# wendongbi/Bridged-GNN

Measured on AMD Instinct MI355X. Metric: aggregated_edges_per_sec_ktgnn_fwd, higher is better.
Workload: dtype f32; 1 GPU; C4 synthetic bridged graph (local) N=1000000 E'=20991058, 2-layer KT-GNN eval fwd F=128 hidden=128 C=2; parallelism=single, execution=eager launches

## Files before the change

bridged_gnn_amd/csrc/bgnn_transform_cls.hip:

```cpp
#include <cstdio>
#include <cstdlib>
#include "bgnn_common.h"
#include "bgnn_transform_params.h"

using bgnn_tf::GemmParams;
using bgnn_tf::MAXH;
using bgnn_tf::f32x16;
using bgnn_tf::tanh_fast;

namespace {

typedef _Float16 h8 __attribute__((ext_vector_type(8)));
typedef _Float16 h4 __attribute__((ext_vector_type(4)));

constexpr int CLS_TARGET_EXP = 10;
constexpr int DK = 128, KB16 = DK / 16, NCT = 4;
constexpr int PIECE = 32 * DK * 2;
constexpr int SLOT = 32 * 36 * 4 + 2 * 32 * 4;
constexpr int T_LD = 36;

__device__ __forceinline__ int chunk_off(int r, int c) { return r * 256 + ((c ^ (r & 15)) << 4); }
__device__ __forceinline__ void pow2_scales(float mx, float& sc, float& inv) {
  int E = (__builtin_bit_cast(int, mx) >> 23) & 0xff;
  E = E < 40 ? 40 : E;
  sc = __builtin_bit_cast(float, (127 + CLS_TARGET_EXP + 127 - E) << 23);
  inv = __builtin_bit_cast(float, (E - CLS_TARGET_EXP) << 23);
}

constexpr int CLS_NW = 4;

__global__ __launch_bounds__(64 * CLS_NW) void cls_stage_kernel(GemmParams p) {
  __shared__ __attribute__((aligned(16))) unsigned char wl[(NCT + 1) * 2 * PIECE];
  __shared__ __attribute__((aligned(16))) unsigned char slots[CLS_NW * SLOT];
  __shared__ __attribute__((aligned(16))) h8 w2lds[NCT][2][2][64];
  __shared__ __attribute__((aligned(16))) float skc[2][32];
  __shared__ __attribute__((aligned(16))) float bias1[DK];
  __shared__ uint32_t wmax[3];
  __shared__ float red[2][DK + 1];
  const int tid = threadIdx.x, lane = tid & 63;
  const int wave = __builtin_amdgcn_readfirstlane(tid >> 6);
  const int fr = lane & 31, fh = lane >> 5;
  const int NC = p.NC;
  const bool din_full = p.Din == DK;
#ifdef CLS_STAMP
  uint32_t st_acc[8] = {0, 0, 0, 0, 0, 0, 0, 0};
  uint32_t st_last = 0;
#define CLS_MARK(k) do { const uint32_t t__ = (uint32_t)__builtin_amdgcn_s_memtime(); st_acc[k] += t__ - st_last; st_last = t__; } while (0)
#else
#define CLS_MARK(k) do { } while (0)
#endif

  if (tid < 3) wmax[tid] = 0u;
  for (int t = tid; t < 2 * (DK + 1); t += 64 * CLS_NW) (&red[0][0])[t] = 0.f;
  if (tid < 32) { skc[0][tid] = tid < p.sk_NC ? p.sk_bias[tid] : 0.f; skc[1][tid] = tid < p.sk_NC ? p.sk_wd[tid] : 0.f; }
  if (tid < DK) bias1[tid] = tid < NC ? p.bias[tid] : 0.f;
  __syncthreads();
  auto src_row = [&](int ct, int r) -> const float* {
    if (ct < NCT) return (32 * ct + r) < NC ? p.Wp + (int64_t)(32 * ct + r) * p.Din : nullptr;
    if (r < p.sk_NC) return p.sk_Wp + (int64_t)r * p.Din;
    if (r >= 24 && ((r - 24) & 3) < 2 * p.sk_heads) return p.sk_g + (int64_t)((r - 24) & 3) * 2 * p.Din;
    return nullptr;
  };
  float mx1 = 0.f, mxs = 0.f;
  for (int it = tid; it < (NCT + 1) * 32 * 16; it += 64 * CLS_NW) {
    const int ct = it / 512, r = (it >> 4) & 31, c = it & 15;
    const float* s = src_row(ct, r);
    float m = 0.f;
    if (s != nullptr) {
#pragma unroll
      for (int e = 0; e < 8; ++e) { const int k = 8 * c + e; m = fmaxf(m, k < p.Din ? fabsf(s[k]) : 0.f); }
    }
    if (ct < NCT) mx1 = fmaxf(mx1, m); else mxs = fmaxf(mxs, m);
  }
  float w2v[NCT][16];
  float mx2 = 0.f;
#pragma unroll
  for (int ct = 0; ct < NCT; ++ct)
#pragma unroll
    for (int r = 0; r < 16; ++r) {
      const int c = 32 * ct + 8 * (r >> 2) + 4 * fh + (r & 3);
      float v = 0.f;
      if (c < NC) {
        if (fr < 8) v = p.w2[(int64_t)fr * NC + c];
        else if (fr < 10) v = p.g2[(int64_t)(fr - 8) * 2 * NC + c];
      }
      w2v[ct][r] = v;
      mx2 = fmaxf(mx2, fabsf(v));
    }
  mx1 = bgnn::group_max<64>(mx1); mxs = bgnn::group_max<64>(mxs); mx2 = bgnn::group_max<64>(mx2);
  if (lane == 0) {
    atomicMax(&wmax[0], __builtin_bit_cast(unsigned, mx1));
    atomicMax(&wmax[1], __builtin_bit_cast(unsigned, mxs));
    atomicMax(&wmax[2], __builtin_bit_cast(unsigned, mx2));
  }
  __syncthreads();
  float scW, cinvW, scS, cinvS, sc2w, cinv2;
  pow2_scales(__builtin_bit_cast(float, wmax[0]), scW, cinvW);
  pow2_scales(__builtin_bit_cast(float, wmax[1]), scS, cinvS);
  pow2_scales(__builtin_bit_cast(float, wmax[2]), sc2w, cinv2);
  for (int it = tid; it < (NCT + 1) * 32 * 16; it += 64 * CLS_NW) {
    const int ct = it / 512, r = (it >> 4) & 31, c = it & 15;
    const float* s = src_row(ct, r);
    const float sc = ct < NCT ? scW : scS;
    h8 hi, lo;
#pragma unroll
    for (int e = 0; e < 8; ++e) {
      const int k = 8 * c + e;
      const float v = (s != nullptr && k < p.Din) ? s[k] : 0.f;
      const _Float16 h = (_Float16)(v * sc);
      hi[e] = h;
      lo[e] = (_Float16)fmaf(v, sc, -(float)h);
    }
    unsigned char* base = wl + (ct * 2) * PIECE + chunk_off(r, c);
    *reinterpret_cast<h8*>(base) = hi;
    *reinterpret_cast<h8*>(base + PIECE) = lo;
  }
  if (wave == 0) {
#pragma unroll
    for (int ct = 0; ct < NCT; ++ct) {
      h8 hh[2], ll[2];
#pragma unroll
      for (int r = 0; r < 16; ++r) {
        const _Float16 h = (_Float16)(w2v[ct][r] * sc2w);
        hh[r >> 3][r & 7] = h;
        ll[r >> 3][r & 7] = (_Float16)fmaf(w2v[ct][r], sc2w, -(float)h);
      }
#pragma unroll
      for (int kb = 0; kb < 2; ++kb) { w2lds[ct][kb][0][lane] = hh[kb]; w2lds[ct][kb][1][lane] = ll[kb]; }
    }
  }
  __syncthreads();

  float* optr[3];
  int hsel[3];
#pragma unroll
  for (int q = 0; q < 3; ++q) {
    const int c = 8 * q + 4 * fh;
    optr[q] = nullptr; hsel[q] = 0;
    if (c < p.sk_NC) {
      const int ld2 = 2 * (int)p.sk_ldh;
      const int h = c / ld2, rem = c % ld2, t = rem >= p.sk_ldh ? 1 : 0;
      float* base = h == 0 ? (t == 0 ? p.sk_out[0][0] : p.sk_out[0][1]) : (t == 0 ? p.sk_out[1][0] : p.sk_out[1][1]);
      optr[q] = base + (rem - t * (int)p.sk_ldh);
      hsel[q] = h * 2 + t;
    }
  }
  float gcs[4];
#pragma unroll
  for (int h = 0; h < 4; ++h) gcs[h] = h < 2 * p.sk_heads ? p.sk_gc[h] : 0.f;

  unsigned char* const sb = slots + wave * SLOT;
  float* const tsc = reinterpret_cast<float*>(sb);
  float* const cfs = reinterpret_cast<float*>(sb + 32 * T_LD * 4);
  const int roff0 = chunk_off(fr, fh);
  auto roff = [&](int kb) { return roff0 ^ (kb << 5); };
  const int64_t ntiles = (p.N + 31) / 32;
  const int64_t stride = (int64_t)gridDim.x * CLS_NW;
  int64_t tile = (int64_t)blockIdx.x * CLS_NW + wave;
  float4 ra[KB16][2];
  uint8_t rmk = 0;
  auto gload = [&](int64_t tl) {
    int64_t r = tl * 32 + fr;
    r = r < p.N ? r : p.N - 1;
    const float* src = p.x + r * p.ldx;
#pragma unroll
    for (int kb = 0; kb < KB16; ++kb)
#pragma unroll
      for (int c = 0; c < 2; ++c) {
        const int k = 16 * kb + 8 * fh + 4 * c;
        ra[kb][c] = *reinterpret_cast<const float4*>(src + (din_full || k < p.Din ? k : 0));
      }
    rmk = p.mask[r];
  };
  float cs_s[NCT], cs_t[NCT], cnt_s = 0.f, cnt_t = 0.f;
#pragma unroll
  for (int ct = 0; ct < NCT; ++ct) cs_s[ct] = cs_t[ct] = 0.f;

  if (tile < ntiles) gload(tile);
  for (; tile < ntiles; tile += stride) {
    CLS_MARK(0);
    const bool sdom = rmk != 0;
    const int64_t row = tile * 32 + fr;
    const bool valid = row < p.N;
    float mx = 0.f;
#pragma unroll
    for (int kb = 0; kb < KB16; ++kb)
#pragma unroll
      for (int c = 0; c < 2; ++c) {
        if (!din_full && 16 * kb + 8 * fh + 4 * c >= p.Din) ra[kb][c] = make_float4(0.f, 0.f, 0.f, 0.f);
        mx = fmaxf(fmaxf(fabsf(ra[kb][c].x), fabsf(ra[kb][c].y)), mx);
        mx = fmaxf(fmaxf(fabsf(ra[kb][c].z), fabsf(ra[kb][c].w)), mx);
      }
    mx = fmaxf(mx, __shfl_xor(mx, 32));
    float scx, s_row;
    pow2_scales(mx, scx, s_row);
    h8 xh[KB16], xl[KB16];
#pragma unroll
    for (int kb = 0; kb < KB16; ++kb)
#pragma unroll
      for (int c = 0; c < 2; ++c) {
        const float f[4] = {ra[kb][c].x, ra[kb][c].y, ra[kb][c].z, ra[kb][c].w};
#pragma unroll
        for (int e = 0; e < 4; ++e) {
          const _Float16 h = (_Float16)(f[e] * scx);
          xh[kb][4 * c + e] = h;
          xl[kb][4 * c + e] = (_Float16)fmaf(f[e], scx, -(float)h);
        }
      }
    const float dom = sdom ? 1.f : 0.f;
    if (fh == 0) {
      cfs[fr] = (valid && sdom) ? 1.f : 0.f;
      cfs[32 + fr] = (valid && !sdom) ? 1.f : 0.f;
      cnt_s += (valid && sdom) ? 1.f : 0.f;
      cnt_t += (valid && !sdom) ? 1.f : 0.f;
    }
    const int64_t tnext = tile + stride < ntiles ? tile + stride : tile;
    gload(tnext);
    __builtin_amdgcn_fence(__ATOMIC_RELEASE, "workgroup", "local");
    constexpr int HK = KB16 / 2;
    h8 wf[2][HK][2];
    auto fetch_w = [&](int hc, int buf) {
      const int op = hc >> 1, half = hc & 1;
      const unsigned char* wb = wl + ((op == 0 ? NCT : op - 1) * 2) * PIECE;
#pragma unroll
      for (int j = 0; j < HK; ++j) {
        wf[buf][j][0] = *reinterpret_cast<const h8*>(wb + roff(HK * half + j));
        wf[buf][j][1] = *reinterpret_cast<const h8*>(wb + PIECE + roff(HK * half + j));
      }
    };
    auto half_chain = [&](int hc, f32x16& acc, auto&& between) {
      if (hc + 1 < 2 * (NCT + 1)) fetch_w(hc + 1, (hc + 1) & 1);
      __builtin_amdgcn_sched_barrier(0);
      const int half = hc & 1, buf = hc & 1;
#pragma unroll
      for (int j = 0; j < HK; ++j) {
        const int kb = HK * half + j;
        acc = __builtin_amdgcn_mfma_f32_32x32x16_f16(wf[buf][j][0], xl[kb], acc, 0, 0, 0);
        acc = __builtin_amdgcn_mfma_f32_32x32x16_f16(wf[buf][j][1], xh[kb], acc, 0, 0, 0);
        acc = __builtin_amdgcn_mfma_f32_32x32x16_f16(wf[buf][j][0], xh[kb], acc, 0, 0, 0);
        between(kb);
      }
    };
    auto nothing = [](int) {};
    CLS_MARK(1);
    fetch_w(0, 0);
    {
      f32x16 acc;
#pragma unroll
      for (int r = 0; r < 16; ++r) acc[r] = 0.f;
      half_chain(0, acc, nothing);
      half_chain(1, acc, nothing);
      CLS_MARK(2);
      const float ss = s_row * cinvS;
      if (valid) {
        float cf = 0.f;
#pragma unroll
        for (int q = 0; q < 3; ++q) {
          if (optr[q] != nullptr) {
            if (q == 0 || hsel[q] != hsel[q - 1]) {
              const bool t1 = hsel[q] & 1;
              const float pre = hsel[q] == 0 ? acc[12] : hsel[q] == 1 ? acc[13] : hsel[q] == 2 ? acc[14] : acc[15];
              const float gcv = hsel[q] == 0 ? gcs[0] : hsel[q] == 1 ? gcs[1] : hsel[q] == 2 ? gcs[2] : gcs[3];
              cf = ((dom != 0.f) != t1) ? tanh_fast(fmaf(pre, ss, gcv)) : 0.f;
              cf = t1 ? cf : -cf;
            }
            const float4 bq = *reinterpret_cast<const float4*>(&skc[0][8 * q + 4 * fh]), wq = *reinterpret_cast<const float4*>(&skc[1][8 * q + 4 * fh]);
            float4 o;
            o.x = fmaf(cf, wq.x, fmaf(acc[4 * q], ss, bq.x));     o.y = fmaf(cf, wq.y, fmaf(acc[4 * q + 1], ss, bq.y));
            o.z = fmaf(cf, wq.z, fmaf(acc[4 * q + 2], ss, bq.z)); o.w = fmaf(cf, wq.w, fmaf(acc[4 * q + 3], ss, bq.w));
            *reinterpret_cast<float4*>(optr[q] + row * p.sk_row_stride) = o;
          }
        }
      }
    }
    float o2[8];
#pragma unroll
    for (int i = 0; i < 8; ++i) o2[i] = 0.f;
    const float sc1 = s_row * cinvW;
    struct Stage2 { float a1[16]; float mx, sc2, inv2; h8 ah[2], al[2]; f32x16 acc2; h8 w2h[2], w2l[2]; };
    auto stage2_step = [&](Stage2& q, int ct, int j) {
      if (j == 0) {
        q.mx = fmaxf(q.mx, __shfl_xor(q.mx, 32));
#pragma unroll
        for (int kb = 0; kb < 2; ++kb) { q.w2h[kb] = w2lds[ct][kb][0][lane]; q.w2l[kb] = w2lds[ct][kb][1][lane]; }
      } else if (j == 1) {
        pow2_scales(q.mx, q.sc2, q.inv2);
#pragma unroll
        for (int r = 0; r < 16; ++r) q.acc2[r] = 0.f;
      } else if (j == 2 || j == 3) {
        const int kb = j - 2;
#pragma unroll
        for (int e = 0; e < 8; ++e) {
          const _Float16 h = (_Float16)(q.a1[8 * kb + e] * q.sc2);
          q.ah[kb][e] = h;
          q.al[kb][e] = (_Float16)fmaf(q.a1[8 * kb + e], q.sc2, -(float)h);
        }
      } else if (j == 4 || j == 5) {
        const int kb = j - 4;
        q.acc2 = __builtin_amdgcn_mfma_f32_32x32x16_f16(q.w2h[kb], q.al[kb], q.acc2, 0, 0, 0);
        q.acc2 = __builtin_amdgcn_mfma_f32_32x32x16_f16(q.w2l[kb], q.ah[kb], q.acc2, 0, 0, 0);
        q.acc2 = __builtin_amdgcn_mfma_f32_32x32x16_f16(q.w2h[kb], q.ah[kb], q.acc2, 0, 0, 0);
      } else if (j == 6) {
#pragma unroll
        for (int r = 0; r < 16; ++r) {
          const float v = tsc[(16 * fh + r) * T_LD + fr];
          cs_s[ct] = fmaf(cfs[16 * fh + r], v, cs_s[ct]);
          cs_t[ct] = fmaf(cfs[32 + 16 * fh + r], v, cs_t[ct]);
        }
      } else {
        const float s2 = q.inv2 * cinv2;
#pragma unroll
        for (int i = 0; i < 8; ++i) o2[i] = fmaf(q.acc2[i], s2, o2[i]);
      }
    };
    Stage2 q2;
    f32x16 acc;
#pragma unroll
    for (int r = 0; r < 16; ++r) acc[r] = 0.f;
    CLS_MARK(3);
    half_chain(2, acc, nothing);
    half_chain(3, acc, nothing);
    CLS_MARK(4);
#pragma unroll
    for (int ct = 0; ct < NCT; ++ct) {
      __builtin_amdgcn_fence(__ATOMIC_RELEASE, "workgroup", "local");
      q2.mx = 0.f;
#pragma unroll
      for (int qq = 0; qq < 4; ++qq) {
        const float4 b4 = *reinterpret_cast<const float4*>(&bias1[32 * ct + 8 * qq + 4 * fh]);
        const float bb[4] = {b4.x, b4.y, b4.z, b4.w};
#pragma unroll
        for (int e = 0; e < 4; ++e) {
          float v = fmaf(acc[4 * qq + e], sc1, bb[e]);
          if (p.relu) v = fmaxf(v, 0.f);
          q2.a1[4 * qq + e] = v;
          q2.mx = fmaxf(q2.mx, fabsf(v));
        }
        *reinterpret_cast<float4*>(&tsc[fr * T_LD + 8 * qq + 4 * fh]) =
            make_float4(q2.a1[4 * qq], q2.a1[4 * qq + 1], q2.a1[4 * qq + 2], q2.a1[4 * qq + 3]);
      }
      CLS_MARK(5);
      if (ct + 1 < NCT) {
#pragma unroll
        for (int r = 0; r < 16; ++r) acc[r] = 0.f;
        half_chain(2 * (ct + 2), acc, [&](int kb) { stage2_step(q2, ct, kb); });
        half_chain(2 * (ct + 2) + 1, acc, [&](int kb) { stage2_step(q2, ct, kb); });
        CLS_MARK(6);
      } else {
#pragma unroll
        for (int j = 0; j < 8; ++j) stage2_step(q2, ct, j);
        CLS_MARK(7);
      }
    }
    if (valid) {
      float* rr = p.raw + row * 12;
      if (fh == 0) {
        *reinterpret_cast<float4*>(rr) = make_float4(o2[0], o2[1], o2[2], o2[3]);
        *reinterpret_cast<float4*>(rr + 8) = make_float4(o2[4], o2[5], 0.f, 0.f);
      } else {
        *reinterpret_cast<float4*>(rr + 4) = make_float4(o2[0], o2[1], o2[2], o2[3]);
      }
    }
  }
#ifdef CLS_STAMP
  if (lane == 0 && p.wd != nullptr) {
    float* o = const_cast<float*>(p.wd) + ((int64_t)blockIdx.x * CLS_NW + wave) * 8;
    for (int k = 0; k < 8; ++k) o[k] = (float)st_acc[k];
  }
  return;
#endif
  if (p.colsum != nullptr) {
#pragma unroll
    for (int ct = 0; ct < NCT; ++ct) {
      const float a = cs_s[ct] + __shfl_xor(cs_s[ct], 32), b = cs_t[ct] + __shfl_xor(cs_t[ct], 32);
      if (fh == 0) {
        unsafeAtomicAdd(&red[0][32 * ct + fr], a);
        unsafeAtomicAdd(&red[1][32 * ct + fr], b);
      }
    }
    {
      float a = cnt_s, b = cnt_t;
#pragma unroll
      for (int m = 32; m >= 1; m >>= 1) { a += __shfl_xor(a, m); b += __shfl_xor(b, m); }
      if (lane == 0) { unsafeAtomicAdd(&red[0][DK], a); unsafeAtomicAdd(&red[1][DK], b); }
    }
    __syncthreads();
    for (int t = tid; t < 2 * (DK + 1); t += 64 * CLS_NW) {
      const int d = t / (DK + 1), c = t % (DK + 1);
      const double v = (double)red[d][c];
      if (c == DK) unsafeAtomicAdd(&p.colsum[2 * NC + d], v);
      else if (c < NC) unsafeAtomicAdd(&p.colsum[d * NC + c], v);
    }
  }
}

}

bool bgnn_tf_cls_supported(const GemmParams& p) {
  if (p.NC != 128 || p.Din > 128 || p.Din <= 64 || (p.Din & 3) || !p.mask || !p.w2 || !p.g2 || !p.raw) return false;
  if (p.sk_NC < 0 || p.sk_NC > 24 || (p.sk_NC & 3) || p.sk_heads < 0 || p.sk_heads > 2) return false;
  if (p.sk_NC > 0 && (!p.sk_Wp || !p.sk_bias || !p.sk_wd || !p.sk_g || !p.sk_gc || (p.sk_ldh & 3) || p.sk_NC != p.sk_heads * 2 * p.sk_ldh)) return false;
  return true;
}

int bgnn_tf_cls_launch(const GemmParams& p, hipStream_t st, int n_cu) {
  if (!bgnn_tf_cls_supported(p)) return BGNN_E_SHAPE;
  const int64_t nt = (p.N + 31) / 32, nb = (nt + CLS_NW - 1) / CLS_NW;
#ifdef CLS_STAMP
  {
    GemmParams q = p;
    static float* dbuf = nullptr;
    if (!dbuf) (void)hipMalloc((void**)&dbuf, sizeof(float) * 256 * 8 * 8);
    q.wd = dbuf;
    const unsigned g = (unsigned)(nb < n_cu ? nb : n_cu);
    hipLaunchKernelGGL(cls_stage_kernel, dim3(g), dim3(64 * CLS_NW), 0, st, q);
    (void)hipDeviceSynchronize();
    static float host[256 * 8 * 8];
    (void)hipMemcpy(host, dbuf, sizeof(float) * g * CLS_NW * 8, hipMemcpyDeviceToHost);
    double acc[8] = {0};
    for (unsigned w = 0; w < g * CLS_NW; ++w) for (int k = 0; k < 8; ++k) acc[k] += host[w * 8 + k];
    const double d = (double)nt;
    fprintf(stderr, "[cls stamp] cycles per tile: loop %.0f convert %.0f skinny-chain %.0f skinny-epilogue %.0f first-chain %.0f activation(x4) %.0f chain+stage2(x3) %.0f last-stage2 %.0f\n",
            acc[0] / d, acc[1] / d, acc[2] / d, acc[3] / d, acc[4] / d, acc[5] / d, acc[6] / d, acc[7] / d);
    return 0;
  }
#endif
  hipLaunchKernelGGL(cls_stage_kernel, dim3((unsigned)(nb < n_cu ? nb : n_cu)), dim3(64 * CLS_NW), 0, st, p);
  BGNN_LAUNCH_CHECK();
  return 0;
}
```

Measured before the change: 49.68 billion edges/s.

## Double waves per block and simplify cls pipeline to cut register pressure

Result: no change. 50.08 billion edges/s (median of 6 runs) (+0.8%).

```diff
diff --git a/bridged_gnn_amd/csrc/bgnn_transform_cls.hip b/bridged_gnn_amd/csrc/bgnn_transform_cls.hip
--- a/bridged_gnn_amd/csrc/bgnn_transform_cls.hip
+++ b/bridged_gnn_amd/csrc/bgnn_transform_cls.hip
@@ -27,7 +27,7 @@
   inv = __builtin_bit_cast(float, (E - CLS_TARGET_EXP) << 23);
 }
 
-constexpr int CLS_NW = 4;
+constexpr int CLS_NW = 8;
 
 __global__ __launch_bounds__(64 * CLS_NW) void cls_stage_kernel(GemmParams p) {
   __shared__ __attribute__((aligned(16))) unsigned char wl[(NCT + 1) * 2 * PIECE];
@@ -156,32 +156,28 @@
   auto roff = [&](int kb) { return roff0 ^ (kb << 5); };
   const int64_t ntiles = (p.N + 31) / 32;
   const int64_t stride = (int64_t)gridDim.x * CLS_NW;
-  int64_t tile = (int64_t)blockIdx.x * CLS_NW + wave;
-  float4 ra[KB16][2];
-  uint8_t rmk = 0;
-  auto gload = [&](int64_t tl) {
-    int64_t r = tl * 32 + fr;
-    r = r < p.N ? r : p.N - 1;
-    const float* src = p.x + r * p.ldx;
-#pragma unroll
-    for (int kb = 0; kb < KB16; ++kb)
-#pragma unroll
-      for (int c = 0; c < 2; ++c) {
-        const int k = 16 * kb + 8 * fh + 4 * c;
-        ra[kb][c] = *reinterpret_cast<const float4*>(src + (din_full || k < p.Din ? k : 0));
-      }
-    rmk = p.mask[r];
-  };
   float cs_s[NCT], cs_t[NCT], cnt_s = 0.f, cnt_t = 0.f;
 #pragma unroll
   for (int ct = 0; ct < NCT; ++ct) cs_s[ct] = cs_t[ct] = 0.f;
 
-  if (tile < ntiles) gload(tile);
-  for (; tile < ntiles; tile += stride) {
+  for (int64_t tile = (int64_t)blockIdx.x * CLS_NW + wave; tile < ntiles; tile += stride) {
     CLS_MARK(0);
-    const bool sdom = rmk != 0;
     const int64_t row = tile * 32 + fr;
     const bool valid = row < p.N;
+    float4 ra[KB16][2];
+    bool sdom;
+    {
+      const int64_t r = valid ? row : p.N - 1;
+      const float* src = p.x + r * p.ldx;
+#pragma unroll
+      for (int kb = 0; kb < KB16; ++kb)
+#pragma unroll
+        for (int c = 0; c < 2; ++c) {
+          const int k = 16 * kb + 8 * fh + 4 * c;
+          ra[kb][c] = *reinterpret_cast<const float4*>(src + (din_full || k < p.Din ? k : 0));
+        }
+      sdom = p.mask[r] != 0;
+    }
     float mx = 0.f;
 #pragma unroll
     for (int kb = 0; kb < KB16; ++kb)
@@ -214,43 +210,39 @@
       cnt_s += (valid && sdom) ? 1.f : 0.f;
       cnt_t += (valid && !sdom) ? 1.f : 0.f;
     }
-    const int64_t tnext = tile + stride < ntiles ? tile + stride : tile;
-    gload(tnext);
-    __builtin_amdgcn_fence(__ATOMIC_RELEASE, "workgroup", "local");
-    constexpr int HK = KB16 / 2;
-    h8 wf[2][HK][2];
-    auto fetch_w = [&](int hc, int buf) {
-      const int op = hc >> 1, half = hc & 1;
-      const unsigned char* wb = wl + ((op == 0 ? NCT : op - 1) * 2) * PIECE;
-#pragma unroll
-      for (int j = 0; j < HK; ++j) {
-        wf[buf][j][0] = *reinterpret_cast<const h8*>(wb + roff(HK * half + j));
-        wf[buf][j][1] = *reinterpret_cast<const h8*>(wb + PIECE + roff(HK * half + j));
+    CLS_MARK(1);
+    auto chain = [&](int op, f32x16& acc) {
+      const unsigned char* wb = wl + (op * 2) * PIECE;
+      h8 wf[2][2][2];
+      auto fetch = [&](int b, int buf) {
+#pragma unroll
+        for (int t = 0; t < 2; ++t) {
+          wf[buf][t][0] = *reinterpret_cast<const h8*>(wb + roff(2 * b + t));
+          wf[buf][t][1] = *reinterpret_cast<const h8*>(wb + PIECE + roff(2 * b + t));
+        }
+      };
+#pragma unroll
+      for (int r = 0; r < 16; ++r) acc[r] = 0.f;
+      fetch(0, 0);
+      fetch(1, 1);
+#pragma unroll
+      for (int b = 0; b < KB16 / 2; ++b) {
+        __builtin_amdgcn_sched_barrier(0);
+#pragma unroll
+        for (int t = 0; t < 2; ++t) {
+          const int kb = 2 * b + t;
+          acc = __builtin_amdgcn_mfma_f32_32x32x16_f16(wf[b & 1][t][0], xl[kb], acc, 0, 0, 0);
+          acc = __builtin_amdgcn_mfma_f32_32x32x16_f16(wf[b & 1][t][1], xh[kb], acc, 0, 0, 0);
+          acc = __builtin_amdgcn_mfma_f32_32x32x16_f16(wf[b & 1][t][0], xh[kb], acc, 0, 0, 0);
+        }
+        __builtin_amdgcn_sched_barrier(0);
+        if (b + 2 < KB16 / 2) fetch(b + 2, b & 1);
       }
     };
-    auto half_chain = [&](int hc, f32x16& acc, auto&& between) {
-      if (hc + 1 < 2 * (NCT + 1)) fetch_w(hc + 1, (hc + 1) & 1);
-      __builtin_amdgcn_sched_barrier(0);
-      const int half = hc & 1, buf = hc & 1;
-#pragma unroll
-      for (int j = 0; j < HK; ++j) {
-        const int kb = HK * half + j;
-        acc = __builtin_amdgcn_mfma_f32_32x32x16_f16(wf[buf][j][0], xl[kb], acc, 0, 0, 0);
-        acc = __builtin_amdgcn_mfma_f32_32x32x16_f16(wf[buf][j][1], xh[kb], acc, 0, 0, 0);
-        acc = __builtin_amdgcn_mfma_f32_32x32x16_f16(wf[buf][j][0], xh[kb], acc, 0, 0, 0);
-        between(kb);
-      }
-    };
-    auto nothing = [](int) {};
-    CLS_MARK(1);
-    fetch_w(0, 0);
+    f32x16 acc;
+    chain(NCT, acc);
+    CLS_MARK(2);
     {
-      f32x16 acc;
-#pragma unroll
-      for (int r = 0; r < 16; ++r) acc[r] = 0.f;
-      half_chain(0, acc, nothing);
-      half_chain(1, acc, nothing);
-      CLS_MARK(2);
       const float ss = s_row * cinvS;
       if (valid) {
         float cf = 0.f;
@@ -273,58 +265,18 @@
         }
       }
     }
+    CLS_MARK(3);
     float o2[8];
 #pragma unroll
     for (int i = 0; i < 8; ++i) o2[i] = 0.f;
     const float sc1 = s_row * cinvW;
-    struct Stage2 { float a1[16]; float mx, sc2, inv2; h8 ah[2], al[2]; f32x16 acc2; h8 w2h[2], w2l[2]; };
-    auto stage2_step = [&](Stage2& q, int ct, int j) {
-      if (j == 0) {
-        q.mx = fmaxf(q.mx, __shfl_xor(q.mx, 32));
-#pragma unroll
-        for (int kb = 0; kb < 2; ++kb) { q.w2h[kb] = w2lds[ct][kb][0][lane]; q.w2l[kb] = w2lds[ct][kb][1][lane]; }
-      } else if (j == 1) {
-        pow2_scales(q.mx, q.sc2, q.inv2);
-#pragma unroll
-        for (int r = 0; r < 16; ++r) q.acc2[r] = 0.f;
-      } else if (j == 2 || j == 3) {
-        const int kb = j - 2;
-#pragma unroll
-        for (int e = 0; e < 8; ++e) {
-          const _Float16 h = (_Float16)(q.a1[8 * kb + e] * q.sc2);
-          q.ah[kb][e] = h;
-          q.al[kb][e] = (_Float16)fmaf(q.a1[8 * kb + e], q.sc2, -(float)h);
-        }
-      } else if (j == 4 || j == 5) {
-        const int kb = j - 4;
-        q.acc2 = __builtin_amdgcn_mfma_f32_32x32x16_f16(q.w2h[kb], q.al[kb], q.acc2, 0, 0, 0);
-        q.acc2 = __builtin_amdgcn_mfma_f32_32x32x16_f16(q.w2l[kb], q.ah[kb], q.acc2, 0, 0, 0);
-        q.acc2 = __builtin_amdgcn_mfma_f32_32x32x16_f16(q.w2h[kb], q.ah[kb], q.acc2, 0, 0, 0);
-      } else if (j == 6) {
-#pragma unroll
-        for (int r = 0; r < 16; ++r) {
-          const float v = tsc[(16 * fh + r) * T_LD + fr];
-          cs_s[ct] = fmaf(cfs[16 * fh + r], v, cs_s[ct]);
-          cs_t[ct] = fmaf(cfs[32 + 16 * fh + r], v, cs_t[ct]);
-        }
-      } else {
-        const float s2 = q.inv2 * cinv2;
-#pragma unroll
-        for (int i = 0; i < 8; ++i) o2[i] = fmaf(q.acc2[i], s2, o2[i]);
-      }
-    };
-    Stage2 q2;
-    f32x16 acc;
-#pragma unroll
-    for (int r = 0; r < 16; ++r) acc[r] = 0.f;
-    CLS_MARK(3);
-    half_chain(2, acc, nothing);
-    half_chain(3, acc, nothing);
-    CLS_MARK(4);
-#pragma unroll
+#pragma unroll 1
     for (int ct = 0; ct < NCT; ++ct) {
+      chain(ct, acc);
+      CLS_MARK(4);
       __builtin_amdgcn_fence(__ATOMIC_RELEASE, "workgroup", "local");
-      q2.mx = 0.f;
+      float a1[16];
+      float amx = 0.f;
 #pragma unroll
       for (int qq = 0; qq < 4; ++qq) {
         const float4 b4 = *reinterpret_cast<const float4*>(&bias1[32 * ct + 8 * qq + 4 * fh]);
@@ -333,24 +285,52 @@
         for (int e = 0; e < 4; ++e) {
           float v = fmaf(acc[4 * qq + e], sc1, bb[e]);
           if (p.relu) v = fmaxf(v, 0.f);
-          q2.a1[4 * qq + e] = v;
-          q2.mx = fmaxf(q2.mx, fabsf(v));
+          a1[4 * qq + e] = v;
+          amx = fmaxf(amx, fabsf(v));
         }
         *reinterpret_cast<float4*>(&tsc[fr * T_LD + 8 * qq + 4 * fh]) =
-            make_float4(q2.a1[4 * qq], q2.a1[4 * qq + 1], q2.a1[4 * qq + 2], q2.a1[4 * qq + 3]);
+            make_float4(a1[4 * qq], a1[4 * qq + 1], a1[4 * qq + 2], a1[4 * qq + 3]);
       }
       CLS_MARK(5);
-      if (ct + 1 < NCT) {
-#pragma unroll
-        for (int r = 0; r < 16; ++r) acc[r] = 0.f;
-        half_chain(2 * (ct + 2), acc, [&](int kb) { stage2_step(q2, ct, kb); });
-        half_chain(2 * (ct + 2) + 1, acc, [&](int kb) { stage2_step(q2, ct, kb); });
-        CLS_MARK(6);
-      } else {
-#pragma unroll
-        for (int j = 0; j < 8; ++j) stage2_step(q2, ct, j);
-        CLS_MARK(7);
-      }
+      amx = fmaxf(amx, __shfl_xor(amx, 32));
+      float sc2, inv2;
+      pow2_scales(amx, sc2, inv2);
+      h8 ah[2], al[2];
+#pragma unroll
+      for (int kb = 0; kb < 2; ++kb)
+#pragma unroll
+        for (int e = 0; e < 8; ++e) {
+          const _Float16 h = (_Float16)(a1[8 * kb + e] * sc2);
+          ah[kb][e] = h;
+          al[kb][e] = (_Float16)fmaf(a1[8 * kb + e], sc2, -(float)h);
+        }
+      f32x16 acc2;
+#pragma unroll
+      for (int r = 0; r < 16; ++r) acc2[r] = 0.f;
+#pragma unroll
+      for (int kb = 0; kb < 2; ++kb) {
+        const h8 w2h = w2lds[ct][kb][0][lane], w2l = w2lds[ct][kb][1][lane];
+        acc2 = __builtin_amdgcn_mfma_f32_32x32x16_f16(w2h, al[kb], acc2, 0, 0, 0);
+        acc2 = __builtin_amdgcn_mfma_f32_32x32x16_f16(w2l, ah[kb], acc2, 0, 0, 0);
+        acc2 = __builtin_amdgcn_mfma_f32_32x32x16_f16(w2h, ah[kb], acc2, 0, 0, 0);
+      }
+      __builtin_amdgcn_fence(__ATOMIC_ACQ_REL, "workgroup", "local");
+#pragma unroll
+      for (int r = 0; r < 16; ++r) {
+        const float v = tsc[(16 * fh + r) * T_LD + fr];
+        cs_s[0] = fmaf(cfs[16 * fh + r], v, cs_s[0]);
+        cs_t[0] = fmaf(cfs[32 + 16 * fh + r], v, cs_t[0]);
+      }
+      {
+        const float ts = cs_s[0], tt = cs_t[0];
+#pragma unroll
+        for (int c = 0; c + 1 < NCT; ++c) { cs_s[c] = cs_s[c + 1]; cs_t[c] = cs_t[c + 1]; }
+        cs_s[NCT - 1] = ts; cs_t[NCT - 1] = tt;
+      }
+      const float s2 = inv2 * cinv2;
+#pragma unroll
+      for (int i = 0; i < 8; ++i) o2[i] = fmaf(acc2[i], s2, o2[i]);
+      CLS_MARK(6);
     }
     if (valid) {
       float* rr = p.raw + row * 12;
@@ -361,6 +341,7 @@
         *reinterpret_cast<float4*>(rr + 4) = make_float4(o2[0], o2[1], o2[2], o2[3]);
       }
     }
+    CLS_MARK(7);
   }
 #ifdef CLS_STAMP
   if (lane == 0 && p.wd != nullptr) {
@@ -420,7 +401,7 @@
     double acc[8] = {0};
     for (unsigned w = 0; w < g * CLS_NW; ++w) for (int k = 0; k < 8; ++k) acc[k] += host[w * 8 + k];
     const double d = (double)nt;
-    fprintf(stderr, "[cls stamp] cycles per tile: loop %.0f convert %.0f skinny-chain %.0f skinny-epilogue %.0f first-chain %.0f activation(x4) %.0f chain+stage2(x3) %.0f last-stage2 %.0f\n",
+    fprintf(stderr, "[cls stamp] cycles per tile and wave: loop %.0f loads+convert %.0f skinny-chain %.0f skinny-epilogue %.0f chains(x4) %.0f activation(x4) %.0f stage2(x4) %.0f stores %.0f\n",
             acc[0] / d, acc[1] / d, acc[2] / d, acc[3] / d, acc[4] / d, acc[5] / d, acc[6] / d, acc[7] / d);
     return 0;
   }
```
